# Atten4Vis/LW-DETR

Measured on AMD Instinct MI355X. Metric: images/sec, higher is better.
Workload: dtype fp16; 1 GPU; LW-DETR-small inference forward + PostProcess, 640x640, batch 32/GPU, fp16, random-init weights (synthetic COCO-shaped input); global_batch=32, per_gpu_batch=32, parallelism=dp1, collective=none, launch_chains=2

## Files before the change

lw-detr_amd/csrc/chain.hip:

```cpp
#include "common.h"
#include <cstdlib>
#include <cstring>

#ifdef LWDETR_CH_TIMING
__device__ unsigned long long g_ch_timing[2][4][16];
#define CH_TS(i) do { if ((blockIdx.x == 0 || blockIdx.x == gridDim.x - 1) && lane == 0) g_ch_timing[blockIdx.x != 0][wave][i] = __builtin_amdgcn_s_memrealtime(); } while (0)
extern "C" int lwdetr_debug_ch_timing(unsigned long long* out) {
    return hipMemcpyFromSymbol(out, HIP_SYMBOL(g_ch_timing), sizeof(g_ch_timing)) == hipSuccess ? 0 : 1;
}
#else
#define CH_TS(i) do {} while (0)
#endif

namespace {

template <typename T> struct Mma32c;
template <> struct Mma32c<f16> {
    static __device__ __forceinline__ f32x16 k16(f16x8 a, f16x8 b, f32x16 c) { return __builtin_amdgcn_mfma_f32_32x32x16_f16(a, b, c, 0, 0, 0); }
};
template <> struct Mma32c<bf16> {
    static __device__ __forceinline__ f32x16 k16(bf16x8 a, bf16x8 b, f32x16 c) { return __builtin_amdgcn_mfma_f32_32x32x16_bf16(a, b, c, 0, 0, 0); }
};
typedef unsigned int cu32x4 __attribute__((ext_vector_type(4)));
typedef float cf32x2 __attribute__((ext_vector_type(2)));
typedef _Float16 cf16x2 __attribute__((ext_vector_type(2)));
typedef __bf16 cbf16x2 __attribute__((ext_vector_type(2)));
template <typename T> struct CPk;
template <> struct CPk<f16> { typedef cf16x2 v2; };
template <> struct CPk<bf16> { typedef cbf16x2 v2; };
template <typename T> __device__ __forceinline__ unsigned cpack2(float a, float b) {
    const cf32x2 v = {a, b};
    return __builtin_bit_cast(unsigned, __builtin_convertvector(v, typename CPk<T>::v2));
}
template <typename T> __device__ __forceinline__ void cunpack2(unsigned w, float& a, float& b) {
    const typename CPk<T>::v2 v = __builtin_bit_cast(typename CPk<T>::v2, w);
    a = to_f32<T>(v[0]); b = to_f32<T>(v[1]);
}
__device__ __forceinline__ cu32x4 crows8(unsigned a0, unsigned a1, unsigned b0, unsigned b1) {
    const auto s0 = __builtin_amdgcn_permlane32_swap(a0, b0, false, false);
    const auto s1 = __builtin_amdgcn_permlane32_swap(a1, b1, false, false);
    return cu32x4{s0[0], s1[0], s0[1], s1[1]};
}

#define CH_VMW(N) asm volatile("s_waitcnt vmcnt(" #N ")" ::: "memory")
__device__ __forceinline__ void ch_wait_le(int n) {
    switch (n) {
#define CH_C(N) case N: CH_VMW(N); break;
        CH_C(1) CH_C(2) CH_C(3) CH_C(4) CH_C(5) CH_C(6) CH_C(7) CH_C(8) CH_C(9) CH_C(10) CH_C(11) CH_C(12) CH_C(13) CH_C(14) CH_C(15)
        CH_C(16) CH_C(17) CH_C(18) CH_C(19) CH_C(20) CH_C(21) CH_C(22) CH_C(23) CH_C(24) CH_C(25) CH_C(26) CH_C(27) CH_C(28) CH_C(29) CH_C(30)
        CH_C(31)
#undef CH_C
        default: CH_VMW(0); break;
    }
}

constexpr int CH_PIECE_B = 4096;
constexpr int CH_RD = 8;

template <int NSLOT>
struct WRing {
    const char* src; unsigned lds0; int np; int issued; int wave; unsigned lane16;
    __device__ __forceinline__ void dma1k(const char* src_uniform, unsigned voff, unsigned lds_dst) {
        const unsigned lo = __builtin_amdgcn_readfirstlane((unsigned)(uintptr_t)src_uniform);
        const unsigned hi = __builtin_amdgcn_readfirstlane((unsigned)((uintptr_t)src_uniform >> 32));
        const char* sp = (const char*)(((uintptr_t)hi << 32) | lo);
        const unsigned m0v = __builtin_amdgcn_readfirstlane(lds_dst);
        asm volatile("s_mov_b32 m0, %0\n\ts_nop 0\n\tglobal_load_lds_dwordx4 %1, %2" :: "s"(m0v), "v"(voff), "s"(sp) : "memory");
    }
    __device__ __forceinline__ void dma_piece(int piece) {
        const unsigned slot = (unsigned)piece % NSLOT;
        dma1k(src + (size_t)piece * CH_PIECE_B, (unsigned)wave * 1024u + lane16, lds0 + slot * CH_PIECE_B + (unsigned)wave * 1024u);
    }
    __device__ __forceinline__ void fill(int first) { for (; issued < first && issued < NSLOT && issued < np; ++issued) dma_piece(issued); }
    template <int STEADY>
    __device__ __forceinline__ void begin_tile(int a, int n) {
        __builtin_amdgcn_sched_barrier(0);
        int b = a + n + 2; b = b < np ? b : np;
        const int v = issued - b;
        if (v == STEADY) asm volatile("s_waitcnt vmcnt(%0)" :: "n"(STEADY) : "memory");
        else ch_wait_le(v);
        asm volatile("s_waitcnt lgkmcnt(0)" ::: "memory");
        __builtin_amdgcn_s_barrier();
        int lim = a + NSLOT; lim = lim < np ? lim : np;
        while (issued < lim) { dma_piece(issued); ++issued; }
        __builtin_amdgcn_sched_barrier(0);
    }

    int vmseq, need, lim; unsigned seq_lds;
#ifdef LWDETR_CH_TIMING
    unsigned long long tt_wait = 0, tt_bar = 0;
#endif
    __device__ __forceinline__ void seq_init(unsigned table_lds_byte_offset) {
        vmseq = 0; need = 0; lim = issued; seq_lds = table_lds_byte_offset;
        for (int i = 0; i < NSLOT; ++i) *(__attribute__((address_space(3))) int*)(uintptr_t)(seq_lds + 4 * i) = 0;
    }
    __device__ __forceinline__ void issue_one() {
        if (issued < lim) {
            dma_piece(issued);
            ++vmseq;
            *(__attribute__((address_space(3))) int*)(uintptr_t)(seq_lds + 4 * ((unsigned)issued % NSLOT)) = vmseq;
            ++issued;
        }
    }
    __device__ __forceinline__ void flush() { while (issued < lim) issue_one(); }
    __device__ __forceinline__ void stores(int k) { vmseq += k; }
    __device__ __forceinline__ void begin_tile_x(int a, int n, int n_next) {
        __builtin_amdgcn_sched_barrier(0);
        flush();
#ifdef LWDETR_CH_TIMING
        const unsigned long long ta = __builtin_amdgcn_s_memrealtime();
#endif
        int allowed = vmseq - need;
        allowed = allowed > 60 ? 60 : allowed & ~3;
        switch (allowed >> 2) {
#define CH_C(N) case N: asm volatile("s_waitcnt vmcnt(%0)" :: "n"(4 * N) : "memory"); break;
            CH_C(1) CH_C(2) CH_C(3) CH_C(4) CH_C(5) CH_C(6) CH_C(7) CH_C(8) CH_C(9) CH_C(10) CH_C(11) CH_C(12) CH_C(13) CH_C(14) CH_C(15)
#undef CH_C
            default: asm volatile("s_waitcnt vmcnt(0)" ::: "memory"); break;
        }
        asm volatile("s_waitcnt lgkmcnt(%0)" :: "n"(CH_RD) : "memory");
#ifdef LWDETR_CH_TIMING
        const unsigned long long tb = __builtin_amdgcn_s_memrealtime();
#endif
        __builtin_amdgcn_s_barrier();
#ifdef LWDETR_CH_TIMING
        tt_wait += tb - ta; tt_bar += __builtin_amdgcn_s_memrealtime() - tb;
#endif
        lim = a + NSLOT; lim = lim < np ? lim : np;
        int q = a + n + n_next + 1; q = q < np - 1 ? q : np - 1;
        need = *(__attribute__((address_space(3))) const int*)(uintptr_t)(seq_lds + 4 * ((unsigned)q % NSLOT));
        flush();
        __builtin_amdgcn_sched_barrier(0);
    }
};

struct EncParams {
    const void* in; long ld_in;
    void* memory;
    void* om; void* cls; long ld_cls; float* cls_max;
    void* values[6]; int nl;
    const unsigned char* rowvalid; const unsigned char* notpad;
    const void* wstream; const float* vec; int np;
    long M;
    int npix, S, lsi;
    int ncls;
    float eps_p, eps_e;
    unsigned mem_bytes, cls_bytes, in_bytes;
};

template <typename T, int D, bool PF, int K5>
__global__ __launch_bounds__(256, 1) void enc_chain_kernel(const EncParams p) {
    typedef typename Vec<T>::v8 V8;
    constexpr int KS = D / 16, NTI = D / 32, PPT = D / 64;
    constexpr int KSI = PF ? K5 / 16 : KS, PPT5 = K5 / 64;
    constexpr int NSLOT = 32;
    constexpr int NCT = 3;
    constexpr int VEC_F = (PF ? 3 * D : 0) + 3 * D + 32 * NCT + 6 * D;
    constexpr int VEC_B = (VEC_F * 4 + 4095) / 4096 * 4096, VEC_DPW = VEC_B / 4096;
    constexpr bool TWO_CHAINS = D == 256 && !PF;
    static_assert(KS % CH_RD == 0 && KSI % CH_RD == 0, "the fragment read-ahead ring must divide every tile");
    extern __shared__ __attribute__((aligned(16))) char smem[];
    const float* vec = (const float*)(smem + NSLOT * CH_PIECE_B);
    const float* b2s = vec; const float* gps = vec + D; const float* bps = vec + 2 * D;
    const float* bes = vec + (PF ? 3 * D : 0); const float* ges = bes + D; const float* bts = ges + D;
    const float* bcs = bts + D; const float* bvs = bcs + 32 * NCT;

    const int tid = threadIdx.x, lane = tid & 63, wave = __builtin_amdgcn_readfirstlane(tid >> 6);
    const int j = lane & 31, h = lane >> 5;
    const unsigned lane16 = lane * 16;
    const unsigned lds0 = (unsigned)(uintptr_t)(__attribute__((address_space(3))) const void*)smem;

    const long t0 = ((long)blockIdx.x * 4 + wave) * 32;
    const long mrow = t0 + j;
    const bool live = mrow < p.M;
    CH_TS(0);
    const long img = live ? mrow / p.npix : 0;
    const long mm = live ? img * p.S + p.lsi + (mrow - img * p.npix) : 0;

    const __amdgpu_buffer_rsrc_t r_in = __builtin_amdgcn_make_buffer_rsrc((void*)p.in, 0, (int)p.in_bytes, 0x00020000);
    const unsigned in_off = live ? (unsigned)(mrow * p.ld_in * 2) : 0x80000000u;
    V8 xin[KSI];
#pragma unroll
    for (int t = 0; t < KSI; ++t)
        xin[t] = __builtin_bit_cast(V8, __builtin_amdgcn_raw_buffer_load_b128(r_in, in_off + (unsigned)((16 * t + 8 * h) * 2), 0, 0));
    const unsigned char rv = live ? p.rowvalid[mm] : 0, npd = live ? p.notpad[mm] : 0;

    WRing<NSLOT> ring;
    ring.src = (const char*)p.wstream; ring.lds0 = lds0; ring.np = p.np; ring.issued = 0; ring.wave = wave; ring.lane16 = lane16;
    {
        const char* vsrc = (const char*)p.vec;
#pragma unroll
        for (int i = 0; i < VEC_DPW; ++i) {
            const unsigned kb = (unsigned)(wave * VEC_DPW + i) * 1024u;
            ring.dma1k(vsrc, kb + lane16, lds0 + NSLOT * CH_PIECE_B + kb);
        }
        ring.fill(2 * (PF ? PPT5 : PPT) + 2);
    }
    __builtin_amdgcn_s_waitcnt(0x0F70);
    ring.seq_init(lds0 + NSLOT * CH_PIECE_B + VEC_B + (unsigned)wave * NSLOT * 4);
    CH_TS(1);
    auto frag = [&](int g) -> V8 {
        return *(const V8*)(smem + (((unsigned)g & (NSLOT * 4 - 1)) << 10) + lane16);
    };
    auto bias16 = [&](const float* src) -> f32x16 {
        f32x16 r;
#pragma unroll
        for (int b = 0; b < 4; ++b) {
            const f32x4 v = *(const f32x4*)(src + 8 * b + 4 * h);
#pragma unroll
            for (int e = 0; e < 4; ++e) r[4 * b + e] = v[e];
        }
        return r;
    };
    const __amdgpu_buffer_rsrc_t r_mem = __builtin_amdgcn_make_buffer_rsrc(p.memory ? p.memory : p.om, 0, p.memory ? (int)p.mem_bytes : 0, 0x00020000);
    const __amdgpu_buffer_rsrc_t r_om = __builtin_amdgcn_make_buffer_rsrc(p.om, 0, (int)p.mem_bytes, 0x00020000);
    const __amdgpu_buffer_rsrc_t r_cls = __builtin_amdgcn_make_buffer_rsrc(p.cls, 0, (int)p.cls_bytes, 0x00020000);
    const unsigned row_off = live ? (unsigned)(mm * D * 2) : 0x80000000u;
    const unsigned cls_off = live ? (unsigned)(mm * p.ld_cls * 2) : 0x80000000u;

    int pc = 0;
    V8 fr[CH_RD];
#ifdef LWDETR_CH_TIMING
    unsigned long long tt_mfma = 0, tt_epi = 0;
#endif
    auto tile = [&](auto& x, auto nf_tag, f32x16 acc) -> f32x16 {
        constexpr int nf = decltype(nf_tag)::value;
        const int g0 = 4 * pc;
        f32x16 acc2 = {};
#pragma unroll
        for (int f = 0; f < nf; ++f) {
            const V8 a = fr[f % CH_RD];
            fr[f % CH_RD] = frag(g0 + f + CH_RD);
            if (TWO_CHAINS && (f & 1)) acc2 = Mma32c<T>::k16(a, x[f], acc2);
            else acc = Mma32c<T>::k16(a, x[f], acc);
            __builtin_amdgcn_sched_barrier(0);
        }
        pc += nf / 4;
        if (TWO_CHAINS) {
#pragma unroll
            for (int e = 0; e < 16; ++e) acc[e] += acc2[e];
        }
        return acc;
    };
    auto layernorm_store = [&](unsigned (&xp)[NTI][8], float s, const float* gam, const float* bet, float eps,
                               const __amdgpu_buffer_rsrc_t& rs, V8 (&xo)[KS]) {
        s += __shfl_xor(s, 32);
        const float mean = s * (1.f / D);
        float v = 0.f;
#pragma unroll
        for (int n = 0; n < NTI; ++n)
#pragma unroll
            for (int d = 0; d < 8; ++d) {
                float v0, v1; cunpack2<T>(xp[n][d], v0, v1);
                v0 -= mean; v1 -= mean;
                v = fmaf(v0, v0, v); v = fmaf(v1, v1, v);
            }
        v += __shfl_xor(v, 32);
        const float rstd = 1.f / sqrtf(v * (1.f / D) + eps);
#pragma unroll
        for (int n = 0; n < NTI; ++n) {
            unsigned w[8];
#pragma unroll
            for (int b = 0; b < 4; ++b) {
                const int c0 = 32 * n + 8 * b + 4 * h;
                const f32x4 g = *(const f32x4*)(gam + c0), be = *(const f32x4*)(bet + c0);
#pragma unroll
                for (int d = 0; d < 2; ++d) {
                    float v0, v1; cunpack2<T>(xp[n][2 * b + d], v0, v1);
                    w[2 * b + d] = cpack2<T>(fmaf((v0 - mean) * rstd, g[2 * d], be[2 * d]), fmaf((v1 - mean) * rstd, g[2 * d + 1], be[2 * d + 1]));
                }
            }
#pragma unroll
            for (int jb = 0; jb < 2; ++jb) {
                const cu32x4 ow = crows8(w[4 * jb], w[4 * jb + 1], w[4 * jb + 2], w[4 * jb + 3]);
                __builtin_amdgcn_raw_buffer_store_b128(ow, rs, row_off + (unsigned)((32 * n + 16 * jb + 8 * h) * 2), 0, 0);
            }
            xo[2 * n] = __builtin_bit_cast(V8, cu32x4{w[0], w[1], w[2], w[3]});
            xo[2 * n + 1] = __builtin_bit_cast(V8, cu32x4{w[4], w[5], w[6], w[7]});
        }
        ring.stores(2 * NTI);
    };

    V8 xf[KS];
    ring.begin_tile_x(0, PF ? PPT5 : PPT, PF ? PPT5 : PPT);
#pragma unroll
    for (int i = 0; i < CH_RD; ++i) fr[i] = frag(i);
    CH_TS(2);
    if constexpr (PF) {
        unsigned xp[NTI][8];
        float s = 0.f;
#pragma unroll
        for (int n = 0; n < NTI; ++n) {
            if (n > 0) ring.begin_tile_x(pc, PPT5, n + 1 < NTI ? PPT5 : PPT);
            const f32x16 acc = tile(xin, std::integral_constant<int, KSI>{}, bias16(b2s + 32 * n));
#pragma unroll
            for (int d = 0; d < 8; ++d) {
                const float a0 = acc[2 * d], a1 = acc[2 * d + 1];
                const unsigned w = cpack2<T>(a0 / (1.f + __expf(-a0)), a1 / (1.f + __expf(-a1)));
                xp[n][d] = w;
                float v0, v1; cunpack2<T>(w, v0, v1);
                s += v0 + v1;
            }
        }
        layernorm_store(xp, s, gps, bps, p.eps_p, r_mem, xf);
    } else {
#pragma unroll
        for (int t = 0; t < KS; ++t) xf[t] = xin[t];
    }
    CH_TS(3);
    {
        const int nvt = p.nl * NTI;
#pragma unroll 1
        for (int vt = 0; vt < nvt; ++vt) {
            if (PF || vt > 0) ring.begin_tile_x(pc, PPT, PPT);
#ifdef LWDETR_CH_TIMING
            const unsigned long long tv0 = __builtin_amdgcn_s_memrealtime();
#endif
            f32x16 acc = tile(xf, std::integral_constant<int, KS>{}, bias16(bvs + 32 * vt));
#ifdef LWDETR_CH_TIMING
            asm volatile("" : "+v"(acc));
            const unsigned long long tv1 = __builtin_amdgcn_s_memrealtime();
#endif
            const int li = vt / NTI, n = vt - li * NTI;
            const __amdgpu_buffer_rsrc_t r_v = __builtin_amdgcn_make_buffer_rsrc(p.values[li], 0, (int)p.mem_bytes, 0x00020000);
            if (!npd) {
#pragma unroll
                for (int e = 0; e < 16; ++e) acc[e] = 0.f;
            }
#pragma unroll
            for (int jb = 0; jb < 2; ++jb) {
                const cu32x4 ow = crows8(cpack2<T>(acc[8 * jb], acc[8 * jb + 1]), cpack2<T>(acc[8 * jb + 2], acc[8 * jb + 3]),
                                         cpack2<T>(acc[8 * jb + 4], acc[8 * jb + 5]), cpack2<T>(acc[8 * jb + 6], acc[8 * jb + 7]));
                __builtin_amdgcn_raw_buffer_store_b128(ow, r_v, row_off + (unsigned)((32 * n + 16 * jb + 8 * h) * 2), 0, 0);
            }
            ring.stores(2);
#ifdef LWDETR_CH_TIMING
            tt_mfma += tv1 - tv0; tt_epi += __builtin_amdgcn_s_memrealtime() - tv1;
#endif
        }
    }
    CH_TS(4);
    {
        if (!rv) {
#pragma unroll
            for (int t = 0; t < KS; ++t) xf[t] = V8{};
        }
        unsigned xp[NTI][8];
        float s = 0.f;
#pragma unroll
        for (int n = 0; n < NTI; ++n) {
            ring.begin_tile_x(pc, PPT, PPT);
            const f32x16 acc = tile(xf, std::integral_constant<int, KS>{}, bias16(bes + 32 * n));
#pragma unroll
            for (int d = 0; d < 8; ++d) {
                const unsigned w = cpack2<T>(acc[2 * d], acc[2 * d + 1]);
                xp[n][d] = w;
                float v0, v1; cunpack2<T>(w, v0, v1);
                s += v0 + v1;
            }
        }
        layernorm_store(xp, s, ges, bts, p.eps_e, r_om, xf);
    }
    CH_TS(5);
    {
        float mx = -INFINITY;
#pragma unroll
        for (int n = 0; n < NCT; ++n) {
            ring.begin_tile_x(pc, PPT, PPT);
            const f32x16 acc = tile(xf, std::integral_constant<int, KS>{}, bias16(bcs + 32 * n));
            unsigned w[8];
#pragma unroll
            for (int d = 0; d < 8; ++d) {
                w[d] = cpack2<T>(acc[2 * d], acc[2 * d + 1]);
                float v0, v1; cunpack2<T>(w[d], v0, v1);
                const int c = 32 * n + 8 * (d >> 1) + 4 * h + 2 * (d & 1);
                if (c < p.ncls) mx = fmaxf(mx, v0);
                if (c + 1 < p.ncls) mx = fmaxf(mx, v1);
            }
#pragma unroll
            for (int jb = 0; jb < 2; ++jb) {
                const cu32x4 ow = crows8(w[4 * jb], w[4 * jb + 1], w[4 * jb + 2], w[4 * jb + 3]);
                __builtin_amdgcn_raw_buffer_store_b128(ow, r_cls, cls_off + (unsigned)((32 * n + 16 * jb + 8 * h) * 2), 0, 0);
            }
            ring.stores(2);
        }
        mx = fmaxf(mx, __shfl_xor(mx, 32));
        if (live && h == 0) p.cls_max[mm] = mx;
    }
    CH_TS(6);
#ifdef LWDETR_CH_TIMING
    if ((blockIdx.x == 0 || blockIdx.x == gridDim.x - 1) && lane == 0) { g_ch_timing[blockIdx.x != 0][wave][13] = ring.tt_wait; g_ch_timing[blockIdx.x != 0][wave][14] = ring.tt_bar;
        g_ch_timing[blockIdx.x != 0][wave][11] = tt_mfma; g_ch_timing[blockIdx.x != 0][wave][12] = tt_epi; }
#endif
}

enum { CS_FULL = 0, CS_SIDE = 1 };
enum { CF_RES = 1, CF_RELU = 2, CF_LN = 4, CF_STORE = 8, CF_ADDQ = 16 };
struct ChainStageK { int kind, nt, flags, ncols, bias_off, gam_off, bet_off; float eps; void* out; long ldo; unsigned out_bytes; };
struct MlpChainParams {
    const void* in; long ld_in; unsigned in_bytes;
    const void* res; long ld_res; unsigned res_bytes;
    const void* qpos; long ld_q; unsigned q_bytes;
    const void* wstream; const float* vec; int vec_dpw; int np; long M; int nst;
    ChainStageK st[6];
};
constexpr int CH_VEC_MAX_B = 16384;

template <typename T, int D, int KS0, bool RES, bool QP>
__global__ __launch_bounds__(256, 1) void mlp_chain_kernel(const MlpChainParams p) {
    typedef typename Vec<T>::v8 V8;
    constexpr int KS = D / 16, NTI = D / 32, PPT = D / 64, PPT0 = KS0 / 4;
    constexpr int NSLOT = 32;
    constexpr bool TWO_CHAINS = false;
    static_assert(KS % CH_RD == 0 && KS0 % CH_RD == 0, "the fragment read-ahead ring must divide every tile");
    extern __shared__ __attribute__((aligned(16))) char smem[];
    const float* vec = (const float*)(smem + NSLOT * CH_PIECE_B);
    const int tid = threadIdx.x, lane = tid & 63, wave = __builtin_amdgcn_readfirstlane(tid >> 6);
    const int j = lane & 31, h = lane >> 5;
    const unsigned lane16 = lane * 16;
    const unsigned lds0 = (unsigned)(uintptr_t)(__attribute__((address_space(3))) const void*)smem;
    const long t0 = ((long)blockIdx.x * 4 + wave) * 32;
    const long mrow = t0 + j;
    const bool live = mrow < p.M;

    const __amdgpu_buffer_rsrc_t r_in = __builtin_amdgcn_make_buffer_rsrc((void*)p.in, 0, (int)p.in_bytes, 0x00020000);
    const unsigned in_off = live ? (unsigned)(mrow * p.ld_in * 2) : 0x80000000u;
    V8 xin[KS0];
#pragma unroll
    for (int t = 0; t < KS0; ++t)
        xin[t] = __builtin_bit_cast(V8, __builtin_amdgcn_raw_buffer_load_b128(r_in, in_off + (unsigned)((16 * t + 8 * h) * 2), 0, 0));
    cu32x4 xr[RES ? NTI : 1][2], xq[QP ? NTI : 1][2];
    if constexpr (RES) {
        const __amdgpu_buffer_rsrc_t r_res = __builtin_amdgcn_make_buffer_rsrc((void*)p.res, 0, (int)p.res_bytes, 0x00020000);
        const unsigned off = live ? (unsigned)(mrow * p.ld_res * 2) : 0x80000000u;
#pragma unroll
        for (int n = 0; n < NTI; ++n)
#pragma unroll
            for (int jb = 0; jb < 2; ++jb) xr[n][jb] = __builtin_amdgcn_raw_buffer_load_b128(r_res, off + (unsigned)((32 * n + 16 * jb + 8 * h) * 2), 0, 0);
    }
    if constexpr (QP) {
        const __amdgpu_buffer_rsrc_t r_q = __builtin_amdgcn_make_buffer_rsrc((void*)p.qpos, 0, (int)p.q_bytes, 0x00020000);
        const unsigned off = live ? (unsigned)(mrow * p.ld_q * 2) : 0x80000000u;
#pragma unroll
        for (int n = 0; n < NTI; ++n)
#pragma unroll
            for (int jb = 0; jb < 2; ++jb) xq[n][jb] = __builtin_amdgcn_raw_buffer_load_b128(r_q, off + (unsigned)((32 * n + 16 * jb + 8 * h) * 2), 0, 0);
    }
    WRing<NSLOT> ring;
    ring.src = (const char*)p.wstream; ring.lds0 = lds0; ring.np = p.np; ring.issued = 0; ring.wave = wave; ring.lane16 = lane16;
    {
        const char* vsrc = (const char*)p.vec;
        for (int i = 0; i < p.vec_dpw; ++i) {
            const unsigned kb = (unsigned)(wave * p.vec_dpw + i) * 1024u;
            ring.dma1k(vsrc, kb + lane16, lds0 + NSLOT * CH_PIECE_B + kb);
        }
        ring.fill(PPT0 + 2 + 4);
    }
    __builtin_amdgcn_s_waitcnt(0x0F70);
    auto frag = [&](int g) -> V8 { return *(const V8*)(smem + (((unsigned)g & (NSLOT * 4 - 1)) << 10) + lane16); };
    auto bias16 = [&](const float* src) -> f32x16 {
        f32x16 r;
#pragma unroll
        for (int b = 0; b < 4; ++b) {
            const f32x4 v = *(const f32x4*)(src + 8 * b + 4 * h);
#pragma unroll
            for (int e = 0; e < 4; ++e) r[4 * b + e] = v[e];
        }
        return r;
    };
    int pc = 0;
    bool first = true;
    V8 fr[CH_RD];
    auto tile = [&](auto& x, auto nf_tag, f32x16 acc) -> f32x16 {
        constexpr int nf = decltype(nf_tag)::value;
        const int g0 = 4 * pc;
        f32x16 acc2 = {};
#pragma unroll
        for (int f = 0; f < nf; ++f) {
            const V8 a = fr[f % CH_RD];
            fr[f % CH_RD] = frag(g0 + f + CH_RD);
            if (TWO_CHAINS && (f & 1)) acc2 = Mma32c<T>::k16(a, x[f], acc2);
            else acc = Mma32c<T>::k16(a, x[f], acc);
            __builtin_amdgcn_sched_barrier(0);
        }
        pc += nf / 4;
        if (TWO_CHAINS) {
#pragma unroll
            for (int e = 0; e < 16; ++e) acc[e] += acc2[e];
        }
        return acc;
    };
    auto next_tile = [&](int n) {
        if (first) first = false;
        else ring.template begin_tile<NSLOT - 2 * PPT - 2>(pc, n);
    };
    V8 xf[KS];
    if constexpr (KS0 == KS) {
#pragma unroll
        for (int t = 0; t < KS; ++t) xf[t] = xin[t];
    }
    ring.template begin_tile<4>(0, PPT0);
#pragma unroll
    for (int i = 0; i < CH_RD; ++i) fr[i] = frag(i);

    auto full = [&](const ChainStageK& st, auto& x, auto nf_tag) {
        constexpr int nf = decltype(nf_tag)::value;
        const float* bsrc = vec + st.bias_off;
        unsigned xp[NTI][8];
        float s = 0.f;
        const bool relu = st.flags & CF_RELU, has_res = RES && (st.flags & CF_RES);
#pragma unroll
        for (int n = 0; n < NTI; ++n) {
            next_tile(nf / 4);
            f32x16 init = bias16(bsrc + 32 * n);
            if constexpr (RES) {
                if (has_res) {
#pragma unroll
                    for (int jb = 0; jb < 2; ++jb) {
                        const cu32x4 own = crows8(xr[n][jb][0], xr[n][jb][1], xr[n][jb][2], xr[n][jb][3]);
#pragma unroll
                        for (int q = 0; q < 4; ++q) {
                            const unsigned ow_ = own[q];
                            float v0, v1; cunpack2<T>(ow_, v0, v1);
                            init[8 * jb + 2 * q] += v0; init[8 * jb + 2 * q + 1] += v1;
                        }
                    }
                }
            }
            const f32x16 acc = tile(x, nf_tag, init);
#pragma unroll
            for (int d = 0; d < 8; ++d) {
                float a0 = acc[2 * d], a1 = acc[2 * d + 1];
                if (relu) { a0 = fmaxf(a0, 0.f); a1 = fmaxf(a1, 0.f); }
                const unsigned w = cpack2<T>(a0, a1);
                xp[n][d] = w;
                float v0, v1; cunpack2<T>(w, v0, v1);
                s += v0 + v1;
            }
        }
        float mean = 0.f, rstd = 1.f;
        const bool ln = st.flags & CF_LN;
        if (ln) {
            s += __shfl_xor(s, 32);
            mean = s * (1.f / D);
            float v = 0.f;
#pragma unroll
            for (int n = 0; n < NTI; ++n)
#pragma unroll
                for (int d = 0; d < 8; ++d) {
                    float v0, v1; cunpack2<T>(xp[n][d], v0, v1);
                    v0 -= mean; v1 -= mean;
                    v = fmaf(v0, v0, v); v = fmaf(v1, v1, v);
                }
            v += __shfl_xor(v, 32);
            rstd = 1.f / sqrtf(v * (1.f / D) + st.eps);
        }
        const float* gam = vec + st.gam_off; const float* bet = vec + st.bet_off;
        const bool store = st.flags & CF_STORE, addq = QP && (st.flags & CF_ADDQ);
        const __amdgpu_buffer_rsrc_t r_out = __builtin_amdgcn_make_buffer_rsrc(store ? st.out : (void*)p.in, 0, store ? (int)st.out_bytes : 0, 0x00020000);
        const unsigned ooff = live ? (unsigned)(mrow * st.ldo * 2) : 0x80000000u;
#pragma unroll
        for (int n = 0; n < NTI; ++n) {
            unsigned w[8];
#pragma unroll
            for (int b = 0; b < 4; ++b) {
                const int c0 = 32 * n + 8 * b + 4 * h;
                if (ln) {
                    const f32x4 g = *(const f32x4*)(gam + c0), be = *(const f32x4*)(bet + c0);
#pragma unroll
                    for (int d = 0; d < 2; ++d) {
                        float v0, v1; cunpack2<T>(xp[n][2 * b + d], v0, v1);
                        w[2 * b + d] = cpack2<T>(fmaf((v0 - mean) * rstd, g[2 * d], be[2 * d]), fmaf((v1 - mean) * rstd, g[2 * d + 1], be[2 * d + 1]));
                    }
                } else {
                    w[2 * b] = xp[n][2 * b]; w[2 * b + 1] = xp[n][2 * b + 1];
                }
            }
            if (store) {
#pragma unroll
                for (int jb = 0; jb < 2; ++jb) {
                    const cu32x4 ow = crows8(w[4 * jb], w[4 * jb + 1], w[4 * jb + 2], w[4 * jb + 3]);
                    __builtin_amdgcn_raw_buffer_store_b128(ow, r_out, ooff + (unsigned)((32 * n + 16 * jb + 8 * h) * 2), 0, 0);
                }
            }
            if constexpr (QP) {
                if (addq) {
#pragma unroll
                    for (int jb = 0; jb < 2; ++jb) {
                        const cu32x4 own = crows8(xq[n][jb][0], xq[n][jb][1], xq[n][jb][2], xq[n][jb][3]);
#pragma unroll
                        for (int q = 0; q < 4; ++q) {
                            const unsigned qw = own[q];
                            float q0, q1, v0, v1; cunpack2<T>(qw, q0, q1); cunpack2<T>(w[4 * jb + q], v0, v1);
                            w[4 * jb + q] = cpack2<T>(v0 + q0, v1 + q1);
                        }
                    }
                }
            }
            xf[2 * n] = __builtin_bit_cast(V8, cu32x4{w[0], w[1], w[2], w[3]});
            xf[2 * n + 1] = __builtin_bit_cast(V8, cu32x4{w[4], w[5], w[6], w[7]});
        }
    };
    auto side = [&](const ChainStageK& st) {
        const __amdgpu_buffer_rsrc_t r_out = __builtin_amdgcn_make_buffer_rsrc(st.out, 0, (int)st.out_bytes, 0x00020000);
        const unsigned ooff = live ? (unsigned)(mrow * st.ldo * 2) : 0x80000000u;
        const bool wide = (st.ldo % 8 == 0) && (st.ncols % 8 == 0);
        const float* bsrc = vec + st.bias_off;
#pragma unroll 1
        for (int vt = 0; vt < st.nt; ++vt) {
            next_tile(PPT);
            const f32x16 acc = tile(xf, std::integral_constant<int, KS>{}, bias16(bsrc + 32 * vt));
            unsigned w[8];
#pragma unroll
            for (int d = 0; d < 8; ++d) w[d] = cpack2<T>(acc[2 * d], acc[2 * d + 1]);
            if (wide) {
#pragma unroll
                for (int jb = 0; jb < 2; ++jb) {
                    const cu32x4 ow = crows8(w[4 * jb], w[4 * jb + 1], w[4 * jb + 2], w[4 * jb + 3]);
                    const int c0 = 32 * vt + 16 * jb + 8 * h;
                    __builtin_amdgcn_raw_buffer_store_b128(ow, r_out, c0 < st.ncols ? ooff + (unsigned)(c0 * 2) : 0x80000000u, 0, 0);
                }
            } else {
#pragma unroll
                for (int b = 0; b < 4; ++b) {
                    const int c0 = 32 * vt + 8 * b + 4 * h;
                    typedef unsigned int cu32x2 __attribute__((ext_vector_type(2)));
                    __builtin_amdgcn_raw_buffer_store_b64(cu32x2{w[2 * b], w[2 * b + 1]}, r_out, c0 < st.ncols ? ooff + (unsigned)(c0 * 2) : 0x80000000u, 0, 0);
                }
            }
        }
    };
#pragma unroll 1
    for (int si = 0; si < p.nst; ++si) {
        const ChainStageK& st = p.st[si];
        if (st.kind == CS_SIDE) side(st);
        else if (KS0 != KS && si == 0) full(st, xin, std::integral_constant<int, KS0>{});
        else full(st, xf, std::integral_constant<int, KS>{});
    }
}

template <typename T, int D, bool PF, int K5>
int launch_enc(const EncParams& p, hipStream_t st) {
    constexpr int NSLOT = 32, NCT = 3;
    constexpr int VEC_F = (PF ? 3 * D : 0) + 3 * D + 32 * NCT + 6 * D;
    constexpr int VEC_B = (VEC_F * 4 + 4095) / 4096 * 4096;
    constexpr size_t lds = (size_t)NSLOT * CH_PIECE_B + VEC_B + 4 * NSLOT * 4;
    static bool attr_done[16] = {};
    int dev = 0;
    if (hipGetDevice(&dev) != hipSuccess || dev < 0 || dev >= 16) return LWDETR_ERR_LAUNCH;
    if (!attr_done[dev]) {
        if (hipFuncSetAttribute((const void*)enc_chain_kernel<T, D, PF, K5>, hipFuncAttributeMaxDynamicSharedMemorySize, (int)lds) != hipSuccess)
            return LWDETR_ERR_LAUNCH;
        attr_done[dev] = true;
    }
    const long grid = (p.M + 127) / 128;
    const double kin = PF ? (double)K5 : 0.0;
    ProfScope ps(KID_CHAIN, 2.0 * p.M * D * (kin + D + 32.0 * NCT + (double)p.nl * D),
                 (double)p.M * 2.0 * ((PF ? K5 + D : D) + D + 96.0 + (double)p.nl * D) + 4.0 * p.M, st);
    hipLaunchKernelGGL((enc_chain_kernel<T, D, PF, K5>), dim3((unsigned)grid), dim3(256), lds, st, p);
    return lwdetr_check_launch();
}

template <typename T>
int dispatch_enc(const EncParams& p, int D, int k5, hipStream_t st) {
    if (D == 256 && k5 == 640) return launch_enc<T, 256, true, 640>(p, st);
    if (D == 256 && k5 == 0) return launch_enc<T, 256, false, 640>(p, st);
    if (D == 384 && k5 == 0) return launch_enc<T, 384, false, 960>(p, st);
    return LWDETR_ERR_UNSUPPORTED;
}

template <typename T, int D>
__global__ __launch_bounds__(256, 1) void mlp_chain_split_kernel(const MlpChainParams p) {
    typedef typename Vec<T>::v8 V8;
    constexpr int KS = D / 16, NTI = D / 32, PPT = D / 64, TPW = NTI / 4;
    constexpr int HALVES = D == 384 ? 2 : 1, PPH = PPT / HALVES, KSH = KS / HALVES;
    constexpr int NSLOT = D == 384 ? 24 : 32;
    static_assert(NTI % 4 == 0 && PPT % HALVES == 0, "tiles split evenly over 4 waves");
    static_assert(2 * 4 * PPH <= NSLOT, "the ring holds two steps (a step's pieces are issued one step ahead)");
    extern __shared__ __attribute__((aligned(16))) char smem[];
    const int vec_b = p.vec_dpw * 4096;
    const float* vec = (const float*)(smem + NSLOT * CH_PIECE_B);
    char* act = smem + NSLOT * CH_PIECE_B + vec_b;
    float* stats = (float*)(act + KS * 1024);
    const int tid = threadIdx.x, lane = tid & 63, wave = __builtin_amdgcn_readfirstlane(tid >> 6);
    const int j = lane & 31, h = lane >> 5;
    const unsigned lane16 = lane * 16;
    const unsigned lds0 = (unsigned)(uintptr_t)(__attribute__((address_space(3))) const void*)smem;
    const long mrow = (long)blockIdx.x * 32 + j;
    const bool live = mrow < p.M;

    const __amdgpu_buffer_rsrc_t r_in = __builtin_amdgcn_make_buffer_rsrc((void*)p.in, 0, (int)p.in_bytes, 0x00020000);
    const unsigned in_off = live ? (unsigned)(mrow * p.ld_in * 2) : 0x80000000u;
    cu32x4 xi[KS / 4];
#pragma unroll
// ... 412 lines not shown
```

Before: 14920 images/sec.

## Group several weight tiles per ring barrier in encoder chain kernel

Replaces the per-tile weight-ring synchronisation (wait plus workgroup barrier before every 32-column tile) with group-level boundaries covering CH_GROUP_PIECES pieces. Several tiles of value projection, encoder output and class head now run between barriers, which cuts the number of s_barrier and vmcnt waits. The DMA flush also moves before the need-table lookup. The cost is a larger in-flight window in the 32-slot ring, so less prefetch slack relative to group size, plus extra timing counters under the debug macro.

```diff
diff --git a/lw-detr_amd/csrc/chain.hip b/lw-detr_amd/csrc/chain.hip
--- a/lw-detr_amd/csrc/chain.hip
+++ b/lw-detr_amd/csrc/chain.hip
@@ -56,6 +56,9 @@
 
 constexpr int CH_PIECE_B = 4096;
 constexpr int CH_RD = 8;
+#ifndef CH_GROUP_PIECES
+#define CH_GROUP_PIECES 12
+#endif
 
 template <int NSLOT>
 struct WRing {
@@ -88,7 +91,7 @@
 
     int vmseq, need, lim; unsigned seq_lds;
 #ifdef LWDETR_CH_TIMING
-    unsigned long long tt_wait = 0, tt_bar = 0;
+    unsigned long long tt_wait = 0, tt_bar = 0, tt_dma = 0, n_bound = 0;
 #endif
     __device__ __forceinline__ void seq_init(unsigned table_lds_byte_offset) {
         vmseq = 0; need = 0; lim = issued; seq_lds = table_lds_byte_offset;
@@ -104,7 +107,7 @@
     }
     __device__ __forceinline__ void flush() { while (issued < lim) issue_one(); }
     __device__ __forceinline__ void stores(int k) { vmseq += k; }
-    __device__ __forceinline__ void begin_tile_x(int a, int n, int n_next) {
+    __device__ __forceinline__ void begin_group(int a, int n, int n_next) {
         __builtin_amdgcn_sched_barrier(0);
         flush();
 #ifdef LWDETR_CH_TIMING
@@ -124,12 +127,16 @@
 #endif
         __builtin_amdgcn_s_barrier();
 #ifdef LWDETR_CH_TIMING
-        tt_wait += tb - ta; tt_bar += __builtin_amdgcn_s_memrealtime() - tb;
+        const unsigned long long tc = __builtin_amdgcn_s_memrealtime();
+        tt_wait += tb - ta; tt_bar += tc - tb;
 #endif
         lim = a + NSLOT; lim = lim < np ? lim : np;
+        flush();
         int q = a + n + n_next + 1; q = q < np - 1 ? q : np - 1;
         need = *(__attribute__((address_space(3))) const int*)(uintptr_t)(seq_lds + 4 * ((unsigned)q % NSLOT));
-        flush();
+#ifdef LWDETR_CH_TIMING
+        tt_dma += __builtin_amdgcn_s_memrealtime() - tc; ++n_bound;
+#endif
         __builtin_amdgcn_sched_barrier(0);
     }
 };
@@ -158,6 +165,8 @@
     constexpr int VEC_F = (PF ? 3 * D : 0) + 3 * D + 32 * NCT + 6 * D;
     constexpr int VEC_B = (VEC_F * 4 + 4095) / 4096 * 4096, VEC_DPW = VEC_B / 4096;
     constexpr bool TWO_CHAINS = D == 256 && !PF;
+    constexpr int GT = CH_GROUP_PIECES / PPT, GP = GT * PPT;
+    static_assert(GT >= 1 && GT <= NTI && 2 * GP + 2 <= NSLOT && (!PF || PPT5 + (PPT5 > GP ? PPT5 : GP) + 2 <= NSLOT), "two neighbouring groups + the read-ahead fit the ring");
     static_assert(KS % CH_RD == 0 && KSI % CH_RD == 0, "the fragment read-ahead ring must divide every tile");
     extern __shared__ __attribute__((aligned(16))) char smem[];
     const float* vec = (const float*)(smem + NSLOT * CH_PIECE_B);
@@ -194,7 +203,7 @@
             const unsigned kb = (unsigned)(wave * VEC_DPW + i) * 1024u;
             ring.dma1k(vsrc, kb + lane16, lds0 + NSLOT * CH_PIECE_B + kb);
         }
-        ring.fill(2 * (PF ? PPT5 : PPT) + 2);
+        ring.fill((PF ? PPT5 : GP) + 2);
     }
     __builtin_amdgcn_s_waitcnt(0x0F70);
     ring.seq_init(lds0 + NSLOT * CH_PIECE_B + VEC_B + (unsigned)wave * NSLOT * 4);
@@ -282,7 +291,9 @@
     };
 
     V8 xf[KS];
-    ring.begin_tile_x(0, PF ? PPT5 : PPT, PF ? PPT5 : PPT);
+    const int nvt = p.nl * NTI;
+    auto vgp = [&](int vt) -> int { const int r = nvt - vt; return (r < GT ? r : GT) * PPT; };
+    ring.begin_group(0, PF ? PPT5 : GP, PF ? PPT5 : vgp(GT));
 #pragma unroll
     for (int i = 0; i < CH_RD; ++i) fr[i] = frag(i);
     CH_TS(2);
@@ -291,7 +302,7 @@
         float s = 0.f;
 #pragma unroll
         for (int n = 0; n < NTI; ++n) {
-            if (n > 0) ring.begin_tile_x(pc, PPT5, n + 1 < NTI ? PPT5 : PPT);
+            if (n > 0) ring.begin_group(pc, PPT5, n + 1 < NTI ? PPT5 : GP);
             const f32x16 acc = tile(xin, std::integral_constant<int, KSI>{}, bias16(b2s + 32 * n));
 #pragma unroll
             for (int d = 0; d < 8; ++d) {
@@ -309,34 +320,38 @@
     }
     CH_TS(3);
     {
-        const int nvt = p.nl * NTI;
 #pragma unroll 1
-        for (int vt = 0; vt < nvt; ++vt) {
-            if (PF || vt > 0) ring.begin_tile_x(pc, PPT, PPT);
+        for (int vg = 0; vg < nvt; vg += GT) {
+            if (PF || vg > 0) ring.begin_group(pc, vgp(vg), vg + GT < nvt ? vgp(vg + GT) : GP);
+#pragma unroll
+            for (int gi = 0; gi < GT; ++gi) {
+                const int vt = vg + gi;
+                if (GT > 1 && vt >= nvt) break;
 #ifdef LWDETR_CH_TIMING
-            const unsigned long long tv0 = __builtin_amdgcn_s_memrealtime();
+                const unsigned long long tv0 = __builtin_amdgcn_s_memrealtime();
 #endif
-            f32x16 acc = tile(xf, std::integral_constant<int, KS>{}, bias16(bvs + 32 * vt));
+                f32x16 acc = tile(xf, std::integral_constant<int, KS>{}, bias16(bvs + 32 * vt));
 #ifdef LWDETR_CH_TIMING
-            asm volatile("" : "+v"(acc));
-            const unsigned long long tv1 = __builtin_amdgcn_s_memrealtime();
+                asm volatile("" : "+v"(acc));
+                const unsigned long long tv1 = __builtin_amdgcn_s_memrealtime();
 #endif
-            const int li = vt / NTI, n = vt - li * NTI;
-            const __amdgpu_buffer_rsrc_t r_v = __builtin_amdgcn_make_buffer_rsrc(p.values[li], 0, (int)p.mem_bytes, 0x00020000);
-            if (!npd) {
-#pragma unroll
-                for (int e = 0; e < 16; ++e) acc[e] = 0.f;
-            }
-#pragma unroll
-            for (int jb = 0; jb < 2; ++jb) {
-                const cu32x4 ow = crows8(cpack2<T>(acc[8 * jb], acc[8 * jb + 1]), cpack2<T>(acc[8 * jb + 2], acc[8 * jb + 3]),
-                                         cpack2<T>(acc[8 * jb + 4], acc[8 * jb + 5]), cpack2<T>(acc[8 * jb + 6], acc[8 * jb + 7]));
-                __builtin_amdgcn_raw_buffer_store_b128(ow, r_v, row_off + (unsigned)((32 * n + 16 * jb + 8 * h) * 2), 0, 0);
-            }
-            ring.stores(2);
+                const int li = vt / NTI, n = vt - li * NTI;
+                const __amdgpu_buffer_rsrc_t r_v = __builtin_amdgcn_make_buffer_rsrc(p.values[li], 0, (int)p.mem_bytes, 0x00020000);
+                if (!npd) {
+#pragma unroll
+                    for (int e = 0; e < 16; ++e) acc[e] = 0.f;
+                }
+#pragma unroll
+                for (int jb = 0; jb < 2; ++jb) {
+                    const cu32x4 ow = crows8(cpack2<T>(acc[8 * jb], acc[8 * jb + 1]), cpack2<T>(acc[8 * jb + 2], acc[8 * jb + 3]),
+                                             cpack2<T>(acc[8 * jb + 4], acc[8 * jb + 5]), cpack2<T>(acc[8 * jb + 6], acc[8 * jb + 7]));
+                    __builtin_amdgcn_raw_buffer_store_b128(ow, r_v, row_off + (unsigned)((32 * n + 16 * jb + 8 * h) * 2), 0, 0);
+                }
+                ring.stores(2);
 #ifdef LWDETR_CH_TIMING
-            tt_mfma += tv1 - tv0; tt_epi += __builtin_amdgcn_s_memrealtime() - tv1;
+                tt_mfma += tv1 - tv0; tt_epi += __builtin_amdgcn_s_memrealtime() - tv1;
 #endif
+            }
         }
     }
     CH_TS(4);
@@ -349,7 +364,7 @@
         float s = 0.f;
 #pragma unroll
         for (int n = 0; n < NTI; ++n) {
-            ring.begin_tile_x(pc, PPT, PPT);
+            if (n % GT == 0) ring.begin_group(pc, (NTI - n < GT ? NTI - n : GT) * PPT, n + GT < NTI ? (NTI - n - GT < GT ? NTI - n - GT : GT) * PPT : (NCT < GT ? NCT : GT) * PPT);
             const f32x16 acc = tile(xf, std::integral_constant<int, KS>{}, bias16(bes + 32 * n));
 #pragma unroll
             for (int d = 0; d < 8; ++d) {
@@ -366,7 +381,7 @@
         float mx = -INFINITY;
 #pragma unroll
         for (int n = 0; n < NCT; ++n) {
-            ring.begin_tile_x(pc, PPT, PPT);
+            if (n % GT == 0) ring.begin_group(pc, (NCT - n < GT ? NCT - n : GT) * PPT, n + GT < NCT ? (NCT - n - GT < GT ? NCT - n - GT : GT) * PPT : 0);
             const f32x16 acc = tile(xf, std::integral_constant<int, KS>{}, bias16(bcs + 32 * n));
             unsigned w[8];
 #pragma unroll
@@ -390,6 +405,7 @@
     CH_TS(6);
 #ifdef LWDETR_CH_TIMING
     if ((blockIdx.x == 0 || blockIdx.x == gridDim.x - 1) && lane == 0) { g_ch_timing[blockIdx.x != 0][wave][13] = ring.tt_wait; g_ch_timing[blockIdx.x != 0][wave][14] = ring.tt_bar;
+        g_ch_timing[blockIdx.x != 0][wave][9] = ring.tt_dma; g_ch_timing[blockIdx.x != 0][wave][10] = ring.n_bound;
         g_ch_timing[blockIdx.x != 0][wave][11] = tt_mfma; g_ch_timing[blockIdx.x != 0][wave][12] = tt_epi; }
 #endif
 }
```

Result: no change. 14950 images/sec, median of 6 (+0.2%).
